# chathurawidanage/harp

Measured on AMD Instinct MI355X. Metric: sec/iteration K-means (N=1e8, d=100, K=1e4), lower is better.
Workload: dtype bf16; 1 GPU; model=kmeans-allreduce, N=100000000, d=100, K=10000, global_batch=100000000, parallelism=dp1

## Files before the change

csrc/kmeans_resolve.hip:

```cpp
#include "common.h"

namespace {

constexpr int KR_RUN = 2048;

template <int KS>
__global__ __launch_bounds__(64) __attribute__((amdgpu_waves_per_eu(3))) void kmeans_resolve_rowsum_kernel(
    const __bf16* __restrict__ X, long ldx, const __bf16* __restrict__ Cm2, const int* __restrict__ perm,
    const int* __restrict__ start, int NG, long n, int* __restrict__ labels, float* __restrict__ sums, int ld) {
  constexpr int DP = KS * 16;
  constexpr int NCB = (DP + 31) / 32;
  constexpr int STRE = NCB * 32 + 8;
  __shared__ __attribute__((aligned(16))) __bf16 tile[32 * STRE];
  __shared__ bf16x8 atile[KS * 64];
  const int lane = threadIdx.x;
  const int c = lane & 31, h = lane >> 5;
  const long j0 = (long)blockIdx.x * KR_RUN;
  if (j0 >= n) return;
  const long j1 = j0 + KR_RUN < n ? j0 + KR_RUN : n;

  for (int i = lane; i < 32 * STRE; i += 64) tile[i] = (__bf16)0.f;
  int lo = 0, hi = NG;
  while (hi - lo > 1) {
    const int mid = (lo + hi) >> 1;
    if (start[mid] <= j0) lo = mid; else hi = mid;
  }
  int k = lo;
  long kend = start[k + 1];
  int kloaded = -1;
  bool dirty = false;
  floatx16 S[NCB];
#pragma unroll
  for (int b = 0; b < NCB; ++b)
#pragma unroll
    for (int q = 0; q < 16; ++q) S[b][q] = 0.f;

  auto pos = [&](long jb) {
    const long j = jb + c;
    return j < j1 ? j : j1 - 1;
  };
  auto load_rows = [&](bf16x8 (&xf)[KS], int p) {
    const bf16x8* row = (const bf16x8*)(X + (long)p * ldx);
#pragma unroll
    for (int s = 0; s < KS; ++s) xf[s] = row[2 * s + h];
  };
  auto flush = [&](int kk) {
    float* o = sums + ((long)kk * 32 + 4 * h) * ld + c;
#pragma unroll
    for (int b = 0; b < NCB; ++b) {
#pragma unroll
      for (int q = 0; q < 16; ++q) {
        const int rq = (q & 3) + 8 * (q >> 2);
// ... 55 lines not shown
      int row = (mq & 3) + 8 * (mq >> 2) + 4 * h;
      const float om = __shfl_xor(m, 32, 64);
      const int orow = __shfl_xor(row, 32, 64);
      if (om < m || (om == m && orow < row)) row = orow;
      if (mine && h == 0) labels[pc] = k * 32 + row;
      const int code = mine ? row : -1;
#pragma unroll
      for (int t = 0; t < 2; ++t) {
        bf16x8 oh;
#pragma unroll
        for (int j = 0; j < 8; ++j) {
          const int r0 = __builtin_amdgcn_readlane(code, 16 * t + j), r1 = __builtin_amdgcn_readlane(code, 16 * t + 8 + j);
          oh[j] = (__bf16)((h ? r1 : r0) == c ? 1.f : 0.f);
        }
        const __bf16* tp = tile + (16 * t + 8 * h) * STRE + c;
#pragma unroll
        for (int b = 0; b < NCB; ++b) {
          bf16x8 xt;
#pragma unroll
          for (int j = 0; j < 8; ++j) xt[j] = tp[j * STRE + 32 * b];
          S[b] = __builtin_amdgcn_mfma_f32_32x32x16_bf16(oh, xt, S[b], 0, 0, 0);
          __builtin_amdgcn_sched_barrier(0);
        }
      }
      dirty = true;
      cur = sub_end;
    }
  }
  if (dirty) flush(k);
}

template <int KS>
int launch_resolve(const void* X, long ldx, const void* Cm2, const int* perm, const int* start, int NG, long n,
                   int* labels, float* sums, int ld, hipStream_t s) {
  const long nblk = (n + KR_RUN - 1) / KR_RUN;
  kmeans_resolve_rowsum_kernel<KS><<<dim3((unsigned)nblk), dim3(64), 0, s>>>(
      (const __bf16*)X, ldx, (const __bf16*)Cm2, perm, start, NG, n, labels, sums, ld);
  return harp_launch_status();
}

}

HARP_EXPORT int harp_kmeans_resolve_rowsum(const void* X, long ldx, const void* Cm2, int dp, const int* perm,
                                           const int* start, int NG, long n, int* labels, float* sums, int ld,
                                           hipStream_t s) {
  if (n <= 0) return n == 0 ? HARP_OK : HARP_EBADARG;
  if (dp <= 0 || dp % 16 || dp > 128 || ldx < dp || ldx % 8 || ld < dp || NG <= 0 || !labels || !sums)
    return HARP_EBADARG;
  switch (dp / 16) {
    case 1: return launch_resolve<1>(X, ldx, Cm2, perm, start, NG, n, labels, sums, ld, s);
    case 2: return launch_resolve<2>(X, ldx, Cm2, perm, start, NG, n, labels, sums, ld, s);
    case 3: return launch_resolve<3>(X, ldx, Cm2, perm, start, NG, n, labels, sums, ld, s);
    case 4: return launch_resolve<4>(X, ldx, Cm2, perm, start, NG, n, labels, sums, ld, s);
    case 5: return launch_resolve<5>(X, ldx, Cm2, perm, start, NG, n, labels, sums, ld, s);
    case 6: return launch_resolve<6>(X, ldx, Cm2, perm, start, NG, n, labels, sums, ld, s);
    case 7: return launch_resolve<7>(X, ldx, Cm2, perm, start, NG, n, labels, sums, ld, s);
    case 8: return launch_resolve<8>(X, ldx, Cm2, perm, start, NG, n, labels, sums, ld, s);
    default: return HARP_EUNSUPPORTED;
  }
}
```

csrc/segsum.hip:

```cpp
#include "common.h"

namespace {

constexpr int SEG = 64;

__global__ __launch_bounds__(256) void label_hist_kernel(const int* __restrict__ lab, long n, int K, long chunk,
                                                         int* __restrict__ H) {
  extern __shared__ __attribute__((aligned(16))) int hist[];
  for (int k = threadIdx.x; k < K; k += blockDim.x) hist[k] = 0;
  __syncthreads();
  const long a = (long)blockIdx.x * chunk;
  long b = a + chunk;
  if (b > n) b = n;
  for (long i = a + threadIdx.x; i < b; i += blockDim.x) atomicAdd(&hist[lab[i]], 1);
  __syncthreads();
  int* row = H + (long)blockIdx.x * K;
  for (int k = threadIdx.x; k < K; k += blockDim.x) row[k] = hist[k];
}

__global__ void colscan1_kernel(int* __restrict__ H, int nchunks, int K, int* __restrict__ T) {
  const int k = blockIdx.x * blockDim.x + threadIdx.x;
  const int s = blockIdx.y;
  if (k >= K) return;
  const int c0 = s * SEG;
  int c1 = c0 + SEG;
  if (c1 > nchunks) c1 = nchunks;
  int run = 0;
  for (int c = c0; c < c1; ++c) {
    const int v = H[(long)c * K + k];
    H[(long)c * K + k] = run;
    run += v;
  }
  T[(long)s * K + k] = run;
}

__global__ void colscan2_kernel(int* __restrict__ T, int nseg, int K, int* __restrict__ counts) {
  const int k = blockIdx.x * blockDim.x + threadIdx.x;
  if (k >= K) return;
  int run = 0;
  for (int s = 0; s < nseg; ++s) {
    const int v = T[(long)s * K + k];
    T[(long)s * K + k] = run;
    run += v;
  }
  counts[k] = run;
}

__global__ __launch_bounds__(1024) void segscan_kernel(const int* __restrict__ counts, int K, int* __restrict__ start) {
  __shared__ int part[1024];
  const int per = (K + 1023) / 1024;
  const int a = threadIdx.x * per;
  int s = 0;
  for (int j = 0; j < per; ++j)
    if (a + j < K) s += counts[a + j];
  part[threadIdx.x] = s;
  __syncthreads();
  for (int off = 1; off < 1024; off <<= 1) {
    const int v = threadIdx.x >= off ? part[threadIdx.x - off] : 0;
    __syncthreads();
    part[threadIdx.x] += v;
    __syncthreads();
  }
  int run = threadIdx.x ? part[threadIdx.x - 1] : 0;
  for (int j = 0; j < per; ++j)
    if (a + j < K) {
      start[a + j] = run;
      run += counts[a + j];
    }
  if (threadIdx.x == 1023) start[K] = part[1023];
}

__device__ __forceinline__ int xcd_contiguous(unsigned b, unsigned nb) {
  const unsigned q = nb / 8, r = nb % 8, x = b % 8;
  return (int)((x < r ? x * (q + 1) : r * (q + 1) + (x - r) * q) + b / 8);
}

__global__ __launch_bounds__(256) void bucket_kernel(const int* __restrict__ lab, long n, int K, long chunk,
                                                     const int* __restrict__ H, const int* __restrict__ T,
                                                     const int* __restrict__ start, int* __restrict__ perm) {
  extern __shared__ __attribute__((aligned(16))) int cur[];
  const int c = xcd_contiguous(blockIdx.x, gridDim.x), s = c / SEG;
  for (int k = threadIdx.x; k < K; k += blockDim.x)
    cur[k] = start[k] + T[(long)s * K + k] + H[(long)c * K + k];
  __syncthreads();
  const long a = (long)c * chunk;
  long b = a + chunk;
  if (b > n) b = n;
  constexpr int U = 8;
  for (long i0 = a + threadIdx.x; i0 < b; i0 += (long)U * blockDim.x) {
    int l[U];
#pragma unroll
    for (int u = 0; u < U; ++u) {
      const long i = i0 + (long)u * blockDim.x;
      l[u] = i < b ? lab[i] : -1;
    }
#pragma unroll
    for (int u = 0; u < U; ++u)
      if (l[u] >= 0) perm[atomicAdd(&cur[l[u]], 1)] = (int)(i0 + (long)u * blockDim.x);
  }
}

template <int LPR, int RUN, int ROWS = 4>
__global__ __launch_bounds__(256) void rowsum_bf16_kernel(const __bf16* __restrict__ X, int dp, long ldx,
                                                          const int* __restrict__ perm,
                                                          const int* __restrict__ start, int K, long n,
                                                          float* __restrict__ sums, int ld) {
  constexpr int SPW = 64 / LPR;
  const int lane = threadIdx.x & 63;
  const int sl = lane % LPR;
  const long slot = ((long)blockIdx.x * blockDim.x + threadIdx.x) / LPR;
  const long j0 = slot * RUN;
  if (j0 >= n) return;
  long j1 = j0 + RUN;
  if (j1 > n) j1 = n;
  const bool active = sl * 8 < dp;
  int lo = 0, hi = K;
  while (hi - lo > 1) {
    const int mid = (lo + hi) >> 1;
    if (start[mid] <= j0) lo = mid; else hi = mid;
// ... 102 lines not shown
        for (int c = 0; c < VEC; ++c)
          v[q][c] = active[c] ? *(const bf16x8*)(X + (long)pj[q] * ldx + (64 * c + lane) * 8) : bf16x8{};
#pragma unroll
      for (int c = 0; c < VEC; ++c)
#pragma unroll
        for (int q = 0; q < ROWS; q += 4)
#pragma unroll
          for (int e = 0; e < 8; ++e)
            acc[c][e] += ((float)v[q][c][e] + (float)v[q + 1][c][e]) + ((float)v[q + 2][c][e] + (float)v[q + 3][c][e]);
    }
    for (; j < stop; ++j) {
      const long r = perm[j];
#pragma unroll
      for (int c = 0; c < VEC; ++c) {
        if (active[c]) {
          const bf16x8 v = *(const bf16x8*)(X + r * ldx + (64 * c + lane) * 8);
#pragma unroll
          for (int e = 0; e < 8; ++e) acc[c][e] += (float)v[e];
        }
      }
    }
  }
  flush(k);
}

}

HARP_EXPORT long harp_bucket_chunk(long n) {
  long c = 65536;
  while (c > 4096 && (n + c - 1) / c < 1536) c >>= 1;
  return c;
}

HARP_EXPORT long harp_bucket_workspace_ints(long n, int K) {
  const long chunk = harp_bucket_chunk(n);
  const long nch = (n + chunk - 1) / chunk;
  const long nseg = (nch + SEG - 1) / SEG;
  return nch * K + nseg * K + K + (K + 1) + n;
}

HARP_EXPORT int harp_bucket_labels(const int* lab, long n, int K, int* ws, long* start_off, long* perm_off,
                                   hipStream_t s) {
  if (n <= 0 || K <= 0 || K > 16384) return HARP_EBADARG;
  const long chunk = harp_bucket_chunk(n);
  const int nch = (int)((n + chunk - 1) / chunk);
  const int nseg = (nch + SEG - 1) / SEG;
  int* H = ws;
  int* T = H + (long)nch * K;
  int* counts = T + (long)nseg * K;
  int* start = counts + K;
  int* perm = start + K + 1;
  *start_off = start - ws;
  *perm_off = perm - ws;
  const size_t lds = (size_t)K * sizeof(int);
  label_hist_kernel<<<dim3(nch), dim3(256), lds, s>>>(lab, n, K, chunk, H);
  colscan1_kernel<<<dim3((K + 255) / 256, nseg), dim3(256), 0, s>>>(H, nch, K, T);
  colscan2_kernel<<<dim3((K + 255) / 256), dim3(256), 0, s>>>(T, nseg, K, counts);
  segscan_kernel<<<dim3(1), dim3(1024), 0, s>>>(counts, K, start);
  bucket_kernel<<<dim3(nch), dim3(256), lds, s>>>(lab, n, K, chunk, H, T, start, perm);
  return harp_launch_status();
}

HARP_EXPORT int harp_bucket_rowsum_bf16(const void* X, int dp, long ldx, const int* perm, const int* start, int K,
                                        long n, float* sums, int ld, hipStream_t s) {
  if (dp % 8 || dp > 1024 || ld < dp || ldx < dp || ldx % 8 || n <= 0) return n == 0 ? HARP_OK : HARP_EBADARG;
  const int lpr_min = dp / 8;
  const __bf16* Xb = (const __bf16*)X;
  constexpr int RUN = 256;
  auto grid = [&](int lpr) { return dim3((unsigned)(((n + RUN - 1) / RUN * lpr + 255) / 256)); };
  if (lpr_min <= 8) rowsum_bf16_kernel<8, RUN><<<grid(8), dim3(256), 0, s>>>(Xb, dp, ldx, perm, start, K, n, sums, ld);
  else if (lpr_min <= 16) rowsum_bf16_kernel<16, RUN, 8><<<grid(16), dim3(256), 0, s>>>(Xb, dp, ldx, perm, start, K, n, sums, ld);
  else if (lpr_min <= 32) rowsum_bf16_kernel<32, RUN><<<grid(32), dim3(256), 0, s>>>(Xb, dp, ldx, perm, start, K, n, sums, ld);
  else if (dp <= 512) rowsum_wide_bf16_kernel<1, RUN><<<grid(64), dim3(256), 0, s>>>(Xb, dp, ldx, perm, start, K, n, sums, ld);
  else rowsum_wide_bf16_kernel<2, RUN><<<grid(64), dim3(256), 0, s>>>(Xb, dp, ldx, perm, start, K, n, sums, ld);
  return harp_launch_status();
}
```

harp_amd/ops/kmeans.py:

```python
from __future__ import annotations

import math
import os
from dataclasses import dataclass
from typing import Optional

import torch

from . import _lib, segment

KP_ALIGN = 128
ONES = 4
DEFAULT_VARIANT = 16
KEYLESS_VARIANT, KEYED_VARIANT = 16, 15
KEYLESS_MAX_DP = 128
RESOLVE_SPAN = 1 << 23


NARROW_MAX_DP = 256
WIDE_ALIGN = 64
WIDE_VARIANT = int(os.environ.get("HARP_KMEANS_WIDE_VARIANT", "0"))


def padded_dim(d: int) -> int:
    dp = (d + ONES + 15) // 16 * 16
    return dp if dp <= NARROW_MAX_DP else (d + ONES + WIDE_ALIGN - 1) // WIDE_ALIGN * WIDE_ALIGN


def padded_k(k: int) -> int:
    return (k + KP_ALIGN - 1) // KP_ALIGN * KP_ALIGN


def row_stride(dp: int) -> int:
    return (dp + 127) // 128 * 128


def pack_points(x: torch.Tensor, device: torch.device | str | None = None) -> torch.Tensor:
    device = torch.device(device) if device is not None else x.device
    n, d = x.shape
    dp = padded_dim(d)
    dt = torch.bfloat16 if device.type == "cuda" else torch.float32
    ld = row_stride(dp) if device.type == "cuda" else dp
    out = torch.zeros((n, ld), dtype=dt, device=device)
    out[:, :d] = x.to(device=device, dtype=dt)
    out[:, d:d + ONES] = 1.0
    return out[:, :dp]


def generate_points(n: int, d: int, lo: float = 0.0, hi: float = 1000.0, seed: int = 0,
# ... 90 lines not shown
    if want_objective and (obj_partial is None or obj_partial.numel() < nblk):
        obj_partial = torch.empty(nblk, dtype=torch.float32, device=dev)
    _lib.check(lib.harp_kmeans_wide_finish(keys.data_ptr(), n, labels.data_ptr(),
                                           obj_partial.data_ptr() if want_objective else None,
                                           min_dist.data_ptr() if min_dist is not None else None,
                                           _lib.stream_ptr(dev)), "kmeans_wide_finish")
    if sums is not None:
        _check_sums(sums, op, dev)
        perm, start = segment.bucket_labels(labels, op.Cm2.shape[0])
        segment.bucket_rowsum(X, perm, start, sums)
    obj = obj_partial[:nblk].double().sum() if want_objective else None
    return labels, obj


def assign(X: torch.Tensor, op: CentroidOperand, sums: Optional[torch.Tensor] = None,
           labels: Optional[torch.Tensor] = None, want_objective: bool = True, variant: int = DEFAULT_VARIANT,
           obj_partial: Optional[torch.Tensor] = None, accumulate: str = "bucket",
           min_dist: Optional[torch.Tensor] = None):
    n, dp = X.shape
    dev = X.device
    if labels is None:
        labels = torch.empty(n, dtype=torch.int32, device=dev)
    if _lib.use_native(X):
        lib = _lib.kernels()
        if dp > NARROW_MAX_DP:
            if accumulate == "atomic":
                raise ValueError("accumulate='atomic' is only fused into the narrow kernel (dp <= "
                                 f"{NARROW_MAX_DP}); the wide path (dp = {dp}) accumulates by bucket")
            return _assign_wide(X, op, sums, labels, want_objective, obj_partial, min_dist)
        keyless = (variant == KEYLESS_VARIANT and dp <= KEYLESS_MAX_DP and sums is not None
                   and accumulate == "bucket" and min_dist is None)
        if variant == KEYLESS_VARIANT and not keyless:
            variant = KEYED_VARIANT
        if dp > 128:
            variant = 4
        elif variant in (14, 15) and dp // 16 == 5:
            variant = 13
        ppb = lib.harp_kmeans_points_per_block(variant)
        if ppb <= 0:
            raise ValueError(f"unknown kmeans kernel variant {variant}")
        nblk = (n + ppb - 1) // ppb
        if want_objective and (obj_partial is None or obj_partial.numel() < nblk):
            obj_partial = torch.empty(nblk, dtype=torch.float32, device=dev)
        if sums is not None:
            _check_sums(sums, op, dev)
        _check_operands(X, op)
        fused = sums if accumulate == "atomic" else None
        bucket = sums is not None and fused is None
        chunks = pipeline_chunks(n, ppb) if bucket else 1
        per = max(1, (nblk + chunks - 1) // chunks) * ppb
        side = _side_stream(dev) if chunks > 1 else None
        main = torch.cuda.current_stream(dev)
        for r0 in range(0, n, per):
            r1 = min(n, r0 + per)
            b0 = r0 // ppb
            st = lib.harp_kmeans_assign(X[r0].data_ptr(), X.stride(0), op.Cm2.data_ptr(), r1 - r0, dp,
                                        swept_k(op), op.d,
                                        labels[r0].data_ptr(), _lib.ptr(fused),
                                        fused.stride(0) if fused is not None else 0,
                                        obj_partial[b0].data_ptr() if want_objective else None,
                                        min_dist[r0].data_ptr() if min_dist is not None else None, variant,
                                        _lib.stream_ptr(dev))
            _lib.check(st, "kmeans_assign")
            if not bucket:
                continue

            def bucket_sum(lab, Xc):
                if keyless:
                    for s0 in range(0, lab.numel(), RESOLVE_SPAN):
                        ls, Xs = lab[s0:s0 + RESOLVE_SPAN], Xc[s0:s0 + RESOLVE_SPAN]
                        perm, start = segment.bucket_labels(ls, swept_k(op) // 32)
                        segment.resolve_rowsum(Xs, op.Cm2, perm, start, ls, sums)
                else:
                    perm, start = segment.bucket_labels(lab, op.Cm2.shape[0])
                    segment.bucket_rowsum(Xc, perm, start, sums)

            if side is None:
                bucket_sum(labels, X)
                continue
            side.wait_stream(main)
            with torch.cuda.stream(side):
                bucket_sum(labels[r0:r1], X[r0:r1])
        if side is not None:
            main.wait_stream(side)
        obj = obj_partial[:nblk].double().sum() if want_objective else None
        return labels, obj
    Xf = X.float()
    d = op.d
    x = Xf[:, :d]
    C = -0.5 * op.Cm2[: op.K, :d].float()
    dist = op.cn[: op.K].unsqueeze(0) - 2.0 * (x @ C.t())
    lab = dist.argmin(1)
    labels.copy_(lab.to(labels.dtype))
    if min_dist is not None:
        min_dist.copy_((dist.gather(1, lab[:, None])[:, 0] + (x * x).sum(1)).to(min_dist.dtype))
    if sums is not None:
        sums[:, : d + 1].index_add_(0, lab, Xf[:, : d + 1])
    obj = None
    if want_objective:
        xs = (x.double() ** 2).sum(1)
        obj = (dist.gather(1, lab[:, None])[:, 0].double() + xs).clamp_min(0).sum()
    return labels, obj


def normalize(sums: torch.Tensor, c: torch.Tensor, d: int, counts: Optional[torch.Tensor] = None) -> torch.Tensor:
# ... 14 lines not shown
```

harp_amd/ops/segment.py:

```python
from __future__ import annotations

import ctypes
import os
from typing import Dict, Tuple

import torch

from . import _lib

_lib.register({
    "harp_bucket_chunk": [_lib.c_long],
    "harp_bucket_workspace_ints": [_lib.c_long, _lib.c_int],
    "harp_bucket_labels": [_lib.c_void_p, _lib.c_long, _lib.c_int, _lib.c_void_p, _lib.c_void_p, _lib.c_void_p,
                           _lib.c_void_p],
    "harp_bucket_rowsum_bf16": [_lib.c_void_p, _lib.c_int, _lib.c_long, _lib.c_void_p, _lib.c_void_p, _lib.c_int,
                                _lib.c_long, _lib.c_void_p, _lib.c_int, _lib.c_void_p],
    "harp_kmeans_resolve_rowsum": [_lib.c_void_p, _lib.c_long, _lib.c_void_p, _lib.c_int, _lib.c_void_p,
                                   _lib.c_void_p, _lib.c_int, _lib.c_long, _lib.c_void_p, _lib.c_void_p, _lib.c_int,
                                   _lib.c_void_p],
})
_WS: Dict[Tuple, torch.Tensor] = {}


def _lib_ret_long(fn):
    fn.restype = ctypes.c_long
    return fn


def bucket_labels(labels: torch.Tensor, K: int) -> Tuple[torch.Tensor, torch.Tensor]:
    n = labels.numel()
    if not _lib.use_native(labels):
        order = torch.argsort(labels.long(), stable=True)
        counts = torch.bincount(labels.long(), minlength=K)
        start = torch.zeros(K + 1, dtype=torch.int64)
        start[1:] = torch.cumsum(counts, 0)
        return order.to(torch.int32), start.to(torch.int32)
    lib = _lib.kernels()
    _lib_ret_long(lib.harp_bucket_workspace_ints)
    need = lib.harp_bucket_workspace_ints(n, K)
    stream = torch.cuda.current_stream(labels.device).cuda_stream
    key = (labels.device, n, K, stream)
    ws = _WS.get(key)
    if ws is None:
        ws = next((w for k, w in _WS.items() if k[0] == labels.device and k[3] == stream and w.numel() >= need),
                  None)
    if ws is None:
        for k in [k for k in _WS if k[3] == stream]:
            del _WS[k]
        ws = torch.empty(need, dtype=torch.int32, device=labels.device)
        _WS[key] = ws
    so, po = ctypes.c_long(0), ctypes.c_long(0)
    st = lib.harp_bucket_labels(labels.data_ptr(), n, K, ws.data_ptr(), ctypes.byref(so), ctypes.byref(po),
                                _lib.stream_ptr(labels.device))
    _lib.check(st, "bucket_labels")
    return ws[po.value:po.value + n], ws[so.value:so.value + K + 1]


SUM_SLICE = min(1024, max(8, int(os.environ.get("HARP_ROWSUM_SLICE", "1024")) // 8 * 8))


def bucket_rowsum(X: torch.Tensor, perm: torch.Tensor, start: torch.Tensor, out: torch.Tensor) -> torch.Tensor:
    K = start.numel() - 1
    if not _lib.use_native(X):
        idx = torch.repeat_interleave(torch.arange(K), (start[1:] - start[:-1]).long())
        out[:K, : X.shape[1]].index_add_(0, idx, X[perm.long()].float())
        return out
    assert X.dtype == torch.bfloat16 and X.stride(1) == 1 and out.dtype == torch.float32 and out.is_contiguous()
    for c0 in range(0, X.shape[1], SUM_SLICE):
        w = min(SUM_SLICE, X.shape[1] - c0)
        st = _lib.kernels().harp_bucket_rowsum_bf16(X[:, c0:].data_ptr(), w, X.stride(0), perm.data_ptr(),
                                                    start.data_ptr(), K, perm.numel(), out[:, c0:].data_ptr(),
                                                    out.stride(0), _lib.stream_ptr(X.device))
        _lib.check(st, "bucket_rowsum")
    return out


def resolve_rowsum(X: torch.Tensor, Cm2: torch.Tensor, perm: torch.Tensor, start: torch.Tensor,
                   labels: torch.Tensor, out: torch.Tensor) -> torch.Tensor:
    NG = start.numel() - 1
    dp = X.shape[1]
    assert X.dtype == torch.bfloat16 and X.stride(1) == 1 and out.dtype == torch.float32 and out.is_contiguous()
    assert Cm2.dtype == torch.bfloat16 and Cm2.is_contiguous() and Cm2.shape[1] == dp and Cm2.shape[0] >= 32 * NG
    assert out.shape[0] >= 32 * NG and labels.dtype == torch.int32 and labels.is_contiguous()
    assert labels.numel() == perm.numel() == X.shape[0]
    st = _lib.kernels().harp_kmeans_resolve_rowsum(X.data_ptr(), X.stride(0), Cm2.data_ptr(), dp, perm.data_ptr(),
                                                   start.data_ptr(), NG, perm.numel(), labels.data_ptr(),
                                                   out.data_ptr(), out.stride(0), _lib.stream_ptr(X.device))
    _lib.check(st, "kmeans_resolve_rowsum")
    return out
```

csrc/kmeans.hip:

```cpp
#include "common.h"

#include <atomic>
#include <type_traits>

namespace {

constexpr float KM_BIG = 1.0e38f;
constexpr int KM_ONES = 4;

__device__ __forceinline__ float keyed(float v, unsigned idx) {
  return __uint_as_float((__float_as_uint(v) & ~0xFu) | idx);
}

template <int KS, int G, int WAVES_, int RG>
struct KMCfg {
  static constexpr int DP = KS * 16;
  static constexpr int CPR = KS * 2;
  static constexpr int TILE = RG * 32;
  static constexpr int WAVES = WAVES_;
  static constexpr int THREADS = WAVES_ * 64;
  static constexpr int TILE_BYTES = TILE * DP * 2;
  static constexpr int DMA_INSTR = TILE * CPR / 64;
  static constexpr int PTS = WAVES_ * G * 32;
  static_assert((TILE * CPR) % 64 == 0, "tile must be whole 1-KiB DMA pieces");
// ... 10 lines not shown
      const int row = q / C::CPR;
      int c = q - row * C::CPR - ((row >> 3) & 1);
      if (c < 0) c += C::CPR;
      unsigned lo = (unsigned)(row * C::CPR + c) * 16u;
      asm("" : "+v"(lo));
      __builtin_amdgcn_global_load_lds((const void __attribute__((address_space(1)))*)(gsrc + (size_t)lo),
                                       (void __attribute__((address_space(3)))*)(lds + j * 1024), 16, 0, 0);
    }
  }
}

constexpr int km_ring_piece_at(int H, int i) {
  constexpr int at[2][4] = {{5, 7, 10, 13}, {6, 9, 11, 14}};
  for (int p = 0; p < 4; ++p)
    if (at[H][p] == i) return p;
  return -1;
}
constexpr int KM_RING_BARRIER_ITEM = 3;

template <int KS, int G, int WAVES, int RG, int PIPE, int PRIO = 0, int KEYLESS = 0, int RING = 0>
__global__ __launch_bounds__(WAVES * 64) void kmeans_assign_kernel(
    const __bf16* __restrict__ X, long ldx, const __bf16* __restrict__ Cm2, long N, int ntiles, int tail_rg,
    int dcount, int* __restrict__ labels, float* __restrict__ sums, int ld_sums, float* __restrict__ obj_partial,
    float* __restrict__ mind, long nblk, unsigned* __restrict__ next_block) {
  using C = KMCfg<KS, G, WAVES, RG>;
  constexpr int NSLOT = RING ? 3 : 2;
  static_assert(!RING || (KEYLESS && PIPE > 0 && G == 4 && RG == 4 && WAVES == 8 && KS <= 8),
                "the ring sweep is written for the keyless 4 x 4-item stage of 8 waves");
  __shared__ __attribute__((aligned(16))) char smem[NSLOT * C::TILE_BYTES + WAVES * 4 + 16];
  if constexpr (PRIO)
    if (__builtin_amdgcn_readfirstlane((int)threadIdx.x) >= WAVES * 32) __builtin_amdgcn_s_setprio(1);

  long b = blockIdx.x;
  while (b < nblk) {
    int tid = threadIdx.x;
    long nb = N;
    asm volatile("" : "+v"(tid), "+s"(nb));
    const int lane = tid & 63, wave = tid >> 6;
    const int r = lane & 31, h = lane >> 5;
    const int srot = (r >> 3) & 1;
    const int swave = __builtin_amdgcn_readfirstlane(wave);
    const long pbase = (b * WAVES + swave) * (G * 32);
    stage_dma<C>(Cm2, 0, smem, swave, lane);
    if constexpr (RING) stage_dma<C>(Cm2, ntiles > 1 ? 1 : 0, smem + C::TILE_BYTES, swave, lane);

    bf16x8 xf[G][KS];
#pragma unroll
    for (int g = 0; g < G; ++g) {
      long p = pbase + g * 32 + r;
      if (p > nb - 1) p = nb - 1;
      const bf16x8* row = (const bf16x8*)(X + p * ldx);
#pragma unroll
      for (int s = 0; s < KS; ++s) xf[g][s] = row[2 * s + h];
    }

    float best[G];
    int bestt[G];
#pragma unroll
    for (int g = 0; g < G; ++g) { best[g] = KM_BIG; bestt[g] = 0; }
    auto tile_argmin = [&](const floatx16& ac, int g, int tg) {
      if constexpr (KEYLESS) {
        float nb = best[g];
#pragma unroll
        for (int q = 0; q < 16; q += 2) nb = fminf(fminf(nb, ac[q]), ac[q + 1]);
        if (nb < best[g]) bestt[g] = tg;
        best[g] = nb;
      } else {
        float m = keyed(ac[0], 0u);
#pragma unroll
        for (int q = 1; q < 16; ++q) m = fminf(m, keyed(ac[q], (unsigned)q));
        if (m < best[g]) { best[g] = m; bestt[g] = tg; }
      }
    };

    int aoff[KS];
#pragma unroll
    for (int s = 0; s < KS; ++s) {
      int cp = 2 * s + h + srot;
      if (cp >= C::CPR) cp -= C::CPR;
      aoff[s] = (r * C::CPR + cp) * 16;
    }
    const int aoff0 = aoff[0], aoffL = aoff[KS - 1] - 32 * (KS - 1);
    auto a_frag = [&](const char* base, int s) {
      return *(const bf16x8*)(base + (s == KS - 1 ? aoffL : aoff0) + 32 * s);
    };

// ... 113 lines not shown
#pragma unroll
            for (int s = 0; s < KS; ++s) an = __builtin_amdgcn_mfma_f32_32x32x16_bf16(af[rg1 & 1][s], xf[g1][s], an, 0, 0, 0);
          }
          tile_argmin(acc[i & 1], g, t * RG + rg);
          if constexpr (PIPE == 2) {
#pragma unroll
            for (int s = 0; s < KS; ++s) {
              __builtin_amdgcn_sched_group_barrier(0x008, 1, 0);
              __builtin_amdgcn_sched_group_barrier(0x002, 4, 0);
            }
          }
        }
      } else
#pragma unroll
      for (int rg = 0; rg < RG; ++rg) {
        if (rg + 1 < RG) {
          const char* nb = buf + (rg + 1) * 32 * C::CPR * 16;
#pragma unroll
          for (int s = 0; s < KS; ++s) af[(rg + 1) & 1][s] = a_frag(nb, s);
        }
        const int tg = t * RG + rg;
#pragma unroll
        for (int g = 0; g < G; ++g) {
          floatx16 acc = {0.f, 0.f, 0.f, 0.f, 0.f, 0.f, 0.f, 0.f, 0.f, 0.f, 0.f, 0.f, 0.f, 0.f, 0.f, 0.f};
#pragma unroll
          for (int s = 0; s < KS; ++s)
            acc = __builtin_amdgcn_mfma_f32_32x32x16_bf16(af[rg & 1][s], xf[g][s], acc, 0, 0, 0);
          tile_argmin(acc, g, tg);
        }
      }
      asm volatile("s_waitcnt vmcnt(0)" ::: "memory");
      __syncthreads();
    }
    if (tail_rg) {
      const int t = ntiles - 1;
      const char* buf = smem + (t % NSLOT) * C::TILE_BYTES;
      for (int rg = 0; rg < tail_rg; ++rg) {
        const char* nb = buf + rg * 32 * C::CPR * 16;
        bf16x8 af[KS];
#pragma unroll
        for (int s = 0; s < KS; ++s) af[s] = a_frag(nb, s);
        const int tg = t * RG + rg;
#pragma unroll
        for (int g = 0; g < G; ++g) {
          floatx16 acc = {0.f, 0.f, 0.f, 0.f, 0.f, 0.f, 0.f, 0.f, 0.f, 0.f, 0.f, 0.f, 0.f, 0.f, 0.f, 0.f};
#pragma unroll
          for (int s = 0; s < KS; ++s) acc = __builtin_amdgcn_mfma_f32_32x32x16_bf16(af[s], xf[g][s], acc, 0, 0, 0);
          tile_argmin(acc, g, tg);
        }
      }
    }

    {
      int tid = threadIdx.x;
      asm volatile("" : "+v"(tid));
      const int lane = tid & 63, wave = tid >> 6, r = lane & 31, h = lane >> 5;
      unsigned* nextw = (unsigned*)(smem + NSLOT * C::TILE_BYTES + WAVES * 4);
      unsigned fetched = 0;
      if (tid == 0) fetched = gridDim.x + atomicAdd(next_block, 1u);
      auto lane_xor = [&](auto v, int o) {
        return __builtin_bit_cast(decltype(v), __builtin_amdgcn_ds_bpermute((lane ^ o) << 2, __builtin_bit_cast(int, v)));
      };
      int lab[G];
      float local_obj = 0.f;
#pragma unroll
      for (int g = 0; g < G; ++g) {
        float xs = 0.f;
#pragma unroll
        for (int s = 0; s < KS; ++s)
#pragma unroll
          for (int j = 0; j < 8; ++j) {
            const float v = (float)xf[g][s][j];
            xs = fmaf(v, v, xs);
          }
        xs += lane_xor(xs, 32);
        xs -= (float)KM_ONES;
        const float ob = lane_xor(best[g], 32);
        const int obt = lane_xor(bestt[g], 32);
        const bool take = KEYLESS ? (ob < best[g] || (ob == best[g] && obt < bestt[g]))
                                  : (h ? (ob <= best[g]) : (ob < best[g]));
        const float bv = take ? ob : best[g];
        const int bt = take ? obt : bestt[g];
        const int hw = take ? (1 - h) : h;
        const unsigned reg = __float_as_uint(bv) & 0xFu;
        const int idx = KEYLESS ? bt : bt * 32 + (int)(reg & 3u) + 8 * (int)(reg >> 2) + 4 * hw;
        lab[g] = idx;
        const long p = pbase + g * 32 + r;
        if (h == 0 && p < nb) {
          labels[p] = idx;
          const float bd = KEYLESS ? bv : __uint_as_float(__float_as_uint(bv) & ~0xFu);
          local_obj += fmaxf(bd + xs, 0.f);
          if (mind) mind[p] = bd + xs;
        }
      }
      if (obj_partial) {
        for (int o = 32; o > 0; o >>= 1) local_obj += lane_xor(local_obj, o);
        float* red = (float*)(smem + NSLOT * C::TILE_BYTES);
        if (lane == 0) red[wave] = local_obj;
        __syncthreads();
        if (tid == 0) {
          float acc = 0.f;
#pragma unroll
          for (int w = 0; w < WAVES; ++w) acc += red[w];
          obj_partial[b] = acc;
        }
      }

      if (!KEYLESS && sums) {
#pragma unroll
        for (int g = 0; g < G; ++g) {
          for (int i = 0; i < 32; ++i) {
            const long p = pbase + g * 32 + i;
            if (p >= nb) break;
            const int l = __shfl(lab[g], i, 64);
            const __bf16* xr = X + p * ldx;
            float* sr = sums + (long)l * ld_sums;
            for (int c = lane; c <= dcount; c += 64) atomicAdd(sr + c, (float)xr[c]);
          }
        }
      }
      if (tid == 0) *nextw = fetched;
      __syncthreads();
      b = (long)(unsigned)__builtin_amdgcn_readfirstlane((int)*nextw);
    }
  }
}

__global__ void kmeans_normalize_kernel(const float* __restrict__ sums, int ld, float* __restrict__ c,
                                        int Kr, int d, float* __restrict__ counts) {
  const int row = blockIdx.x * (blockDim.x >> 6) + (threadIdx.x >> 6);
  const int lane = threadIdx.x & 63;
  if (row >= Kr) return;
  const float cnt = sums[(long)row * ld + d];
  if (counts && lane == 0) counts[row] = cnt;
  if (cnt > 0.f) {
    const float inv = 1.0f / cnt;
    for (int j = lane; j < d; j += 64) c[(long)row * d + j] = sums[(long)row * ld + j] * inv;
  }
}

__global__ void kmeans_prepare_kernel(const float* __restrict__ c, int K, int d, int Kp, int dp,
                                      __bf16* __restrict__ Cm2, float* __restrict__ cn) {
  const int row = blockIdx.x * (blockDim.x >> 6) + (threadIdx.x >> 6);
  const int lane = threadIdx.x & 63;
  if (row >= Kp) return;
  float s = 0.f;
  for (int j = lane; j < d; j += 64) {
    float v = row < K ? c[(long)row * d + j] : 0.f;
    const float bf = (float)(__bf16)v;
    s = fmaf(bf, bf, s);
    Cm2[(long)row * dp + j] = (__bf16)(-2.0f * bf);
  }
  s = wave_sum(s);
  if (row >= K) s = KM_BIG;
  const __bf16 hi = (__bf16)s;
  const float r1 = s - (float)hi;
// ... 559 lines not shown
```

Before: 0.1336 s/iter.

## Bucket and resolve all label spans in single batched kernel launches

Replaces the Python loop over RESOLVE_SPAN chunks, which launched the five bucketing kernels plus one resolve kernel per span, with span-aware kernels that process every span in one launch. Each resolve block indexes its span's start offsets, and the scan kernels get a per-span grid dimension. The span also shrinks from 2^23 to 2^20 so buckets stay local to smaller windows. This cuts launch and host overhead and may improve locality of gathered rows. In exchange it adds more per-span start tables, more partial bucket flushes and atomics at span boundaries, and extra workspace.

```diff
diff --git a/csrc/kmeans_resolve.hip b/csrc/kmeans_resolve.hip
--- a/csrc/kmeans_resolve.hip
+++ b/csrc/kmeans_resolve.hip
@@ -7,7 +7,8 @@
 template <int KS>
 __global__ __launch_bounds__(64) __attribute__((amdgpu_waves_per_eu(3))) void kmeans_resolve_rowsum_kernel(
     const __bf16* __restrict__ X, long ldx, const __bf16* __restrict__ Cm2, const int* __restrict__ perm,
-    const int* __restrict__ start, int NG, long n, int* __restrict__ labels, float* __restrict__ sums, int ld) {
+    const int* __restrict__ start, int NG, long n, int span_shift, int* __restrict__ labels,
+    float* __restrict__ sums, int ld) {
   constexpr int DP = KS * 16;
   constexpr int NCB = (DP + 31) / 32;
   constexpr int STRE = NCB * 32 + 8;
@@ -18,6 +19,7 @@
   const long j0 = (long)blockIdx.x * KR_RUN;
   if (j0 >= n) return;
   const long j1 = j0 + KR_RUN < n ? j0 + KR_RUN : n;
+  start += (j0 >> span_shift) * (NG + 1);
 
   for (int i = lane; i < 32 * STRE; i += 64) tile[i] = (__bf16)0.f;
   int lo = 0, hi = NG;
@@ -139,30 +141,40 @@
 
 template <int KS>
 int launch_resolve(const void* X, long ldx, const void* Cm2, const int* perm, const int* start, int NG, long n,
-                   int* labels, float* sums, int ld, hipStream_t s) {
+                   int span_shift, int* labels, float* sums, int ld, hipStream_t s) {
   const long nblk = (n + KR_RUN - 1) / KR_RUN;
   kmeans_resolve_rowsum_kernel<KS><<<dim3((unsigned)nblk), dim3(64), 0, s>>>(
-      (const __bf16*)X, ldx, (const __bf16*)Cm2, perm, start, NG, n, labels, sums, ld);
+      (const __bf16*)X, ldx, (const __bf16*)Cm2, perm, start, NG, n, span_shift, labels, sums, ld);
   return harp_launch_status();
 }
 
 }
 
+HARP_EXPORT int harp_kmeans_resolve_run() { return KR_RUN; }
+
+HARP_EXPORT int harp_kmeans_resolve_rowsum_spans(const void* X, long ldx, const void* Cm2, int dp, const int* perm,
+                                                 const int* start, int NG, long n, long span, int* labels,
+                                                 float* sums, int ld, hipStream_t s) {
+  if (n <= 0) return n == 0 ? HARP_OK : HARP_EBADARG;
+  if (dp <= 0 || dp % 16 || dp > 128 || ldx < dp || ldx % 8 || ld < dp || NG <= 0 || !labels || !sums)
+    return HARP_EBADARG;
+  if (span < KR_RUN || (span & (span - 1))) return HARP_EBADARG;
+  const int sh = __builtin_ctzl((unsigned long)span);
+  switch (dp / 16) {
+    case 1: return launch_resolve<1>(X, ldx, Cm2, perm, start, NG, n, sh, labels, sums, ld, s);
+    case 2: return launch_resolve<2>(X, ldx, Cm2, perm, start, NG, n, sh, labels, sums, ld, s);
+    case 3: return launch_resolve<3>(X, ldx, Cm2, perm, start, NG, n, sh, labels, sums, ld, s);
+    case 4: return launch_resolve<4>(X, ldx, Cm2, perm, start, NG, n, sh, labels, sums, ld, s);
+    case 5: return launch_resolve<5>(X, ldx, Cm2, perm, start, NG, n, sh, labels, sums, ld, s);
+    case 6: return launch_resolve<6>(X, ldx, Cm2, perm, start, NG, n, sh, labels, sums, ld, s);
+    case 7: return launch_resolve<7>(X, ldx, Cm2, perm, start, NG, n, sh, labels, sums, ld, s);
+    case 8: return launch_resolve<8>(X, ldx, Cm2, perm, start, NG, n, sh, labels, sums, ld, s);
+    default: return HARP_EUNSUPPORTED;
+  }
+}
+
 HARP_EXPORT int harp_kmeans_resolve_rowsum(const void* X, long ldx, const void* Cm2, int dp, const int* perm,
                                            const int* start, int NG, long n, int* labels, float* sums, int ld,
                                            hipStream_t s) {
-  if (n <= 0) return n == 0 ? HARP_OK : HARP_EBADARG;
-  if (dp <= 0 || dp % 16 || dp > 128 || ldx < dp || ldx % 8 || ld < dp || NG <= 0 || !labels || !sums)
-    return HARP_EBADARG;
-  switch (dp / 16) {
-    case 1: return launch_resolve<1>(X, ldx, Cm2, perm, start, NG, n, labels, sums, ld, s);
-    case 2: return launch_resolve<2>(X, ldx, Cm2, perm, start, NG, n, labels, sums, ld, s);
-    case 3: return launch_resolve<3>(X, ldx, Cm2, perm, start, NG, n, labels, sums, ld, s);
-    case 4: return launch_resolve<4>(X, ldx, Cm2, perm, start, NG, n, labels, sums, ld, s);
-    case 5: return launch_resolve<5>(X, ldx, Cm2, perm, start, NG, n, labels, sums, ld, s);
-    case 6: return launch_resolve<6>(X, ldx, Cm2, perm, start, NG, n, labels, sums, ld, s);
-    case 7: return launch_resolve<7>(X, ldx, Cm2, perm, start, NG, n, labels, sums, ld, s);
-    case 8: return launch_resolve<8>(X, ldx, Cm2, perm, start, NG, n, labels, sums, ld, s);
-    default: return HARP_EUNSUPPORTED;
-  }
+  return harp_kmeans_resolve_rowsum_spans(X, ldx, Cm2, dp, perm, start, NG, n, 1L << 62, labels, sums, ld, s);
 }
diff --git a/csrc/segsum.hip b/csrc/segsum.hip
--- a/csrc/segsum.hip
+++ b/csrc/segsum.hip
@@ -3,6 +3,20 @@
 namespace {
 
 constexpr int SEG = 64;
+
+struct SpanGeom {
+  long chunk;
+  int nch;
+  int cps;
+  int sps;
+  int spans;
+};
+
+__host__ __device__ inline long ceil_pow2(long v) {
+  long p = 1;
+  while (p < v) p <<= 1;
+  return p;
+}
 
 __global__ __launch_bounds__(256) void label_hist_kernel(const int* __restrict__ lab, long n, int K, long chunk,
                                                          int* __restrict__ H) {
@@ -18,13 +32,15 @@
   for (int k = threadIdx.x; k < K; k += blockDim.x) row[k] = hist[k];
 }
 
-__global__ void colscan1_kernel(int* __restrict__ H, int nchunks, int K, int* __restrict__ T) {
+__global__ void colscan1_kernel(int* __restrict__ H, SpanGeom g, int K, int* __restrict__ T) {
   const int k = blockIdx.x * blockDim.x + threadIdx.x;
   const int s = blockIdx.y;
   if (k >= K) return;
-  const int c0 = s * SEG;
+  const int j = s / g.sps;
+  const int c0 = j * g.cps + (s % g.sps) * SEG;
   int c1 = c0 + SEG;
-  if (c1 > nchunks) c1 = nchunks;
+  if (c1 > (j + 1) * g.cps) c1 = (j + 1) * g.cps;
+  if (c1 > g.nch) c1 = g.nch;
   int run = 0;
   for (int c = c0; c < c1; ++c) {
     const int v = H[(long)c * K + k];
@@ -37,6 +53,8 @@
 __global__ void colscan2_kernel(int* __restrict__ T, int nseg, int K, int* __restrict__ counts) {
   const int k = blockIdx.x * blockDim.x + threadIdx.x;
   if (k >= K) return;
+  T += (long)blockIdx.y * nseg * K;
+  counts += (long)blockIdx.y * K;
   int run = 0;
   for (int s = 0; s < nseg; ++s) {
     const int v = T[(long)s * K + k];
@@ -46,8 +64,12 @@
   counts[k] = run;
 }
 
-__global__ __launch_bounds__(1024) void segscan_kernel(const int* __restrict__ counts, int K, int* __restrict__ start) {
+__global__ __launch_bounds__(1024) void segscan_kernel(const int* __restrict__ counts, int K, long span,
+                                                       int* __restrict__ start) {
   __shared__ int part[1024];
+  counts += (long)blockIdx.x * K;
+  start += (long)blockIdx.x * (K + 1);
+  const int base = (int)(blockIdx.x * span);
   const int per = (K + 1023) / 1024;
   const int a = threadIdx.x * per;
   int s = 0;
@@ -61,13 +83,13 @@
     part[threadIdx.x] += v;
     __syncthreads();
   }
-  int run = threadIdx.x ? part[threadIdx.x - 1] : 0;
+  int run = base + (threadIdx.x ? part[threadIdx.x - 1] : 0);
   for (int j = 0; j < per; ++j)
     if (a + j < K) {
       start[a + j] = run;
       run += counts[a + j];
     }
-  if (threadIdx.x == 1023) start[K] = part[1023];
+  if (threadIdx.x == 1023) start[K] = base + part[1023];
 }
 
 __device__ __forceinline__ int xcd_contiguous(unsigned b, unsigned nb) {
@@ -75,16 +97,17 @@
   return (int)((x < r ? x * (q + 1) : r * (q + 1) + (x - r) * q) + b / 8);
 }
 
-__global__ __launch_bounds__(256) void bucket_kernel(const int* __restrict__ lab, long n, int K, long chunk,
+__global__ __launch_bounds__(256) void bucket_kernel(const int* __restrict__ lab, long n, int K, SpanGeom g,
                                                      const int* __restrict__ H, const int* __restrict__ T,
                                                      const int* __restrict__ start, int* __restrict__ perm) {
   extern __shared__ __attribute__((aligned(16))) int cur[];
-  const int c = xcd_contiguous(blockIdx.x, gridDim.x), s = c / SEG;
+  const int c = xcd_contiguous(blockIdx.x, gridDim.x);
+  const int j = c / g.cps, s = j * g.sps + (c % g.cps) / SEG;
   for (int k = threadIdx.x; k < K; k += blockDim.x)
-    cur[k] = start[k] + T[(long)s * K + k] + H[(long)c * K + k];
+    cur[k] = start[(long)j * (K + 1) + k] + T[(long)s * K + k] + H[(long)c * K + k];
   __syncthreads();
-  const long a = (long)c * chunk;
-  long b = a + chunk;
+  const long a = (long)c * g.chunk;
+  long b = a + g.chunk;
   if (b > n) b = n;
   constexpr int U = 8;
   for (long i0 = a + threadIdx.x; i0 < b; i0 += (long)U * blockDim.x) {
@@ -253,33 +276,62 @@
   return c;
 }
 
+namespace {
+
+SpanGeom span_geom(long n, long span) {
+  SpanGeom g;
+  g.chunk = harp_bucket_chunk(n < span ? n : span);
+  if (g.chunk > span) g.chunk = span;
+  g.nch = (int)((n + g.chunk - 1) / g.chunk);
+  const long cps = span / g.chunk;
+  g.cps = (int)(cps < g.nch ? cps : g.nch);
+  g.sps = (g.cps + SEG - 1) / SEG;
+  g.spans = (int)((n + span - 1) / span);
+  return g;
+}
+
+long workspace_ints(const SpanGeom& g, long n, int K) {
+  return (long)g.nch * K + (long)g.spans * g.sps * K + (long)g.spans * K + (long)g.spans * (K + 1) + n;
+}
+
+bool span_ok(long span) { return span > 0 && (span & (span - 1)) == 0; }
+
+}
+
 HARP_EXPORT long harp_bucket_workspace_ints(long n, int K) {
-  const long chunk = harp_bucket_chunk(n);
-  const long nch = (n + chunk - 1) / chunk;
-  const long nseg = (nch + SEG - 1) / SEG;
-  return nch * K + nseg * K + K + (K + 1) + n;
-}
-
-HARP_EXPORT int harp_bucket_labels(const int* lab, long n, int K, int* ws, long* start_off, long* perm_off,
-                                   hipStream_t s) {
-  if (n <= 0 || K <= 0 || K > 16384) return HARP_EBADARG;
-  const long chunk = harp_bucket_chunk(n);
-  const int nch = (int)((n + chunk - 1) / chunk);
-  const int nseg = (nch + SEG - 1) / SEG;
+  return n > 0 ? workspace_ints(span_geom(n, ceil_pow2(n)), n, K) : 0;
+}
+
+HARP_EXPORT long harp_bucket_spans_workspace_ints(long n, int K, long span) {
+  if (!span_ok(span)) return -1;
+  return n > 0 ? workspace_ints(span_geom(n, span), n, K) : 0;
+}
+
+HARP_EXPORT int harp_bucket_labels_spans(const int* lab, long n, int K, long span, int* ws, long* start_off,
+                                         long* perm_off, hipStream_t s) {
+  if (n <= 0 || n > 0x7fffffffL || K <= 0 || K > 16384 || !span_ok(span)) return HARP_EBADARG;
+  const SpanGeom g = span_geom(n, span);
+  if ((long)g.spans * g.sps > 65535) return HARP_EUNSUPPORTED;
   int* H = ws;
-  int* T = H + (long)nch * K;
-  int* counts = T + (long)nseg * K;
-  int* start = counts + K;
-  int* perm = start + K + 1;
+  int* T = H + (long)g.nch * K;
+  int* counts = T + (long)g.spans * g.sps * K;
+  int* start = counts + (long)g.spans * K;
+  int* perm = start + (long)g.spans * (K + 1);
   *start_off = start - ws;
   *perm_off = perm - ws;
   const size_t lds = (size_t)K * sizeof(int);
-  label_hist_kernel<<<dim3(nch), dim3(256), lds, s>>>(lab, n, K, chunk, H);
-  colscan1_kernel<<<dim3((K + 255) / 256, nseg), dim3(256), 0, s>>>(H, nch, K, T);
-  colscan2_kernel<<<dim3((K + 255) / 256), dim3(256), 0, s>>>(T, nseg, K, counts);
-  segscan_kernel<<<dim3(1), dim3(1024), 0, s>>>(counts, K, start);
-  bucket_kernel<<<dim3(nch), dim3(256), lds, s>>>(lab, n, K, chunk, H, T, start, perm);
+  const unsigned kb = (K + 255) / 256;
+  label_hist_kernel<<<dim3(g.nch), dim3(256), lds, s>>>(lab, n, K, g.chunk, H);
+  colscan1_kernel<<<dim3(kb, g.spans * g.sps), dim3(256), 0, s>>>(H, g, K, T);
+  colscan2_kernel<<<dim3(kb, g.spans), dim3(256), 0, s>>>(T, g.sps, K, counts);
+  segscan_kernel<<<dim3(g.spans), dim3(1024), 0, s>>>(counts, K, span, start);
+  bucket_kernel<<<dim3(g.nch), dim3(256), lds, s>>>(lab, n, K, g, H, T, start, perm);
   return harp_launch_status();
+}
+
+HARP_EXPORT int harp_bucket_labels(const int* lab, long n, int K, int* ws, long* start_off, long* perm_off,
+                                   hipStream_t s) {
+  return harp_bucket_labels_spans(lab, n, K, ceil_pow2(n > 0 ? n : 1), ws, start_off, perm_off, s);
 }
 
 HARP_EXPORT int harp_bucket_rowsum_bf16(const void* X, int dp, long ldx, const int* perm, const int* start, int K,
diff --git a/harp_amd/ops/kmeans.py b/harp_amd/ops/kmeans.py
--- a/harp_amd/ops/kmeans.py
+++ b/harp_amd/ops/kmeans.py
@@ -14,7 +14,7 @@
 DEFAULT_VARIANT = 16
 KEYLESS_VARIANT, KEYED_VARIANT = 16, 15
 KEYLESS_MAX_DP = 128
-RESOLVE_SPAN = 1 << 23
+RESOLVE_SPAN = 1 << 20
 
 
 NARROW_MAX_DP = 256
@@ -171,6 +171,9 @@
                    and accumulate == "bucket" and min_dist is None)
         if variant == KEYLESS_VARIANT and not keyless:
             variant = KEYED_VARIANT
+        span = RESOLVE_SPAN
+        if keyless and (span < segment.resolve_run() or span & (span - 1)):
+            raise ValueError(f"RESOLVE_SPAN must be a power of two of at least {segment.resolve_run()}, got {span}")
         if dp > 128:
             variant = 4
         elif variant in (14, 15) and dp // 16 == 5:
@@ -206,10 +209,8 @@
 
             def bucket_sum(lab, Xc):
                 if keyless:
-                    for s0 in range(0, lab.numel(), RESOLVE_SPAN):
-                        ls, Xs = lab[s0:s0 + RESOLVE_SPAN], Xc[s0:s0 + RESOLVE_SPAN]
-                        perm, start = segment.bucket_labels(ls, swept_k(op) // 32)
-                        segment.resolve_rowsum(Xs, op.Cm2, perm, start, ls, sums)
+                    perm, start = segment.bucket_labels(lab, swept_k(op) // 32, span=span)
+                    segment.resolve_rowsum(Xc, op.Cm2, perm, start, lab, sums, span=span)
                 else:
                     perm, start = segment.bucket_labels(lab, op.Cm2.shape[0])
                     segment.bucket_rowsum(Xc, perm, start, sums)
diff --git a/harp_amd/ops/segment.py b/harp_amd/ops/segment.py
--- a/harp_amd/ops/segment.py
+++ b/harp_amd/ops/segment.py
@@ -2,7 +2,7 @@
 
 import ctypes
 import os
-from typing import Dict, Tuple
+from typing import Dict, Optional, Tuple
 
 import torch
 
@@ -13,11 +13,18 @@
     "harp_bucket_workspace_ints": [_lib.c_long, _lib.c_int],
     "harp_bucket_labels": [_lib.c_void_p, _lib.c_long, _lib.c_int, _lib.c_void_p, _lib.c_void_p, _lib.c_void_p,
                            _lib.c_void_p],
+    "harp_bucket_spans_workspace_ints": [_lib.c_long, _lib.c_int, _lib.c_long],
+    "harp_bucket_labels_spans": [_lib.c_void_p, _lib.c_long, _lib.c_int, _lib.c_long, _lib.c_void_p, _lib.c_void_p,
+                                 _lib.c_void_p, _lib.c_void_p],
     "harp_bucket_rowsum_bf16": [_lib.c_void_p, _lib.c_int, _lib.c_long, _lib.c_void_p, _lib.c_void_p, _lib.c_int,
                                 _lib.c_long, _lib.c_void_p, _lib.c_int, _lib.c_void_p],
     "harp_kmeans_resolve_rowsum": [_lib.c_void_p, _lib.c_long, _lib.c_void_p, _lib.c_int, _lib.c_void_p,
                                    _lib.c_void_p, _lib.c_int, _lib.c_long, _lib.c_void_p, _lib.c_void_p, _lib.c_int,
                                    _lib.c_void_p],
+    "harp_kmeans_resolve_run": [],
+    "harp_kmeans_resolve_rowsum_spans": [_lib.c_void_p, _lib.c_long, _lib.c_void_p, _lib.c_int, _lib.c_void_p,
+                                         _lib.c_void_p, _lib.c_int, _lib.c_long, _lib.c_long, _lib.c_void_p,
+                                         _lib.c_void_p, _lib.c_int, _lib.c_void_p],
 })
 _WS: Dict[Tuple, torch.Tensor] = {}
 
@@ -27,33 +34,45 @@
     return fn
 
 
-def bucket_labels(labels: torch.Tensor, K: int) -> Tuple[torch.Tensor, torch.Tensor]:
+def _one_span(n: int) -> int:
+    return 1 << max(0, n - 1).bit_length()
+
+
+def bucket_labels(labels: torch.Tensor, K: int, span: Optional[int] = None) -> Tuple[torch.Tensor, torch.Tensor]:
     n = labels.numel()
+    if span is not None and (span <= 0 or span & (span - 1)):
+        raise ValueError(f"span must be a power of two, got {span}")
     if not _lib.use_native(labels):
-        order = torch.argsort(labels.long(), stable=True)
-        counts = torch.bincount(labels.long(), minlength=K)
-        start = torch.zeros(K + 1, dtype=torch.int64)
-        start[1:] = torch.cumsum(counts, 0)
-        return order.to(torch.int32), start.to(torch.int32)
+        w = n if span is None else span
+        lab = labels.long()
+        order = torch.cat([s0 + torch.argsort(lab[s0:s0 + w], stable=True) for s0 in range(0, n, w)])
+        counts = torch.stack([torch.bincount(lab[s0:s0 + w], minlength=K) for s0 in range(0, n, w)])
+        start = torch.zeros((counts.shape[0], K + 1), dtype=torch.int64)
+        start[:, 1:] = torch.cumsum(counts, 1)
+        start += torch.arange(0, n, w)[:, None]
+        return order.to(torch.int32), (start[0] if span is None else start).to(torch.int32)
     lib = _lib.kernels()
-    _lib_ret_long(lib.harp_bucket_workspace_ints)
-    need = lib.harp_bucket_workspace_ints(n, K)
+    _lib_ret_long(lib.harp_bucket_spans_workspace_ints)
+    cspan = _one_span(n) if span is None else span
+    spans = (n + cspan - 1) // cspan
+    need = lib.harp_bucket_spans_workspace_ints(n, K, cspan)
     stream = torch.cuda.current_stream(labels.device).cuda_stream
-    key = (labels.device, n, K, stream)
+    key = (labels.device, n, K, cspan, stream)
     ws = _WS.get(key)
     if ws is None:
-        ws = next((w for k, w in _WS.items() if k[0] == labels.device and k[3] == stream and w.numel() >= need),
+        ws = next((w for k, w in _WS.items() if k[0] == labels.device and k[-1] == stream and w.numel() >= need),
                   None)
     if ws is None:
-        for k in [k for k in _WS if k[3] == stream]:
+        for k in [k for k in _WS if k[-1] == stream]:
             del _WS[k]
         ws = torch.empty(need, dtype=torch.int32, device=labels.device)
         _WS[key] = ws
     so, po = ctypes.c_long(0), ctypes.c_long(0)
-    st = lib.harp_bucket_labels(labels.data_ptr(), n, K, ws.data_ptr(), ctypes.byref(so), ctypes.byref(po),
-                                _lib.stream_ptr(labels.device))
+    st = lib.harp_bucket_labels_spans(labels.data_ptr(), n, K, cspan, ws.data_ptr(), ctypes.byref(so),
+                                      ctypes.byref(po), _lib.stream_ptr(labels.device))
     _lib.check(st, "bucket_labels")
-    return ws[po.value:po.value + n], ws[so.value:so.value + K + 1]
+    start = ws[so.value:so.value + spans * (K + 1)]
+    return ws[po.value:po.value + n], (start if span is None else start.view(spans, K + 1))
 
 
 SUM_SLICE = min(1024, max(8, int(os.environ.get("HARP_ROWSUM_SLICE", "1024")) // 8 * 8))
@@ -75,16 +94,23 @@
     return out
 
 
+def resolve_run() -> int:
+    return _lib.kernels().harp_kmeans_resolve_run()
+
+
 def resolve_rowsum(X: torch.Tensor, Cm2: torch.Tensor, perm: torch.Tensor, start: torch.Tensor,
-                   labels: torch.Tensor, out: torch.Tensor) -> torch.Tensor:
-    NG = start.numel() - 1
-    dp = X.shape[1]
+                   labels: torch.Tensor, out: torch.Tensor, span: Optional[int] = None) -> torch.Tensor:
+    n, dp = X.shape
+    NG = start.shape[-1] - 1
+    cspan = _one_span(max(n, resolve_run())) if span is None else span
     assert X.dtype == torch.bfloat16 and X.stride(1) == 1 and out.dtype == torch.float32 and out.is_contiguous()
     assert Cm2.dtype == torch.bfloat16 and Cm2.is_contiguous() and Cm2.shape[1] == dp and Cm2.shape[0] >= 32 * NG
     assert out.shape[0] >= 32 * NG and labels.dtype == torch.int32 and labels.is_contiguous()
-    assert labels.numel() == perm.numel() == X.shape[0]
-    st = _lib.kernels().harp_kmeans_resolve_rowsum(X.data_ptr(), X.stride(0), Cm2.data_ptr(), dp, perm.data_ptr(),
-                                                   start.data_ptr(), NG, perm.numel(), labels.data_ptr(),
-                                                   out.data_ptr(), out.stride(0), _lib.stream_ptr(X.device))
+    assert labels.numel() == perm.numel() == n
+    assert start.is_contiguous() and start.numel() == (n + cspan - 1) // cspan * (NG + 1)
+    st = _lib.kernels().harp_kmeans_resolve_rowsum_spans(X.data_ptr(), X.stride(0), Cm2.data_ptr(), dp,
+                                                         perm.data_ptr(), start.data_ptr(), NG, n, cspan,
+                                                         labels.data_ptr(), out.data_ptr(), out.stride(0),
+                                                         _lib.stream_ptr(X.device))
     _lib.check(st, "kmeans_resolve_rowsum")
     return out
```

New measurement: 0.1327 s/iter (median of 6 runs). Within noise of the previous version (-0.7%).

## Prefetch next block's points and first centroid tiles during epilogue

Applied to the files above, without the earlier changes.

In the persistent assign kernel, the next block index is now fetched with a relaxed atomic before the tail tiles are processed. The epilogue then starts the DMA of the first centroid tiles and the loads of the next block's X rows while the current block's labels and objective are still being written. This hides the per-block startup latency of the X loads and tile staging. It also skips the squared-norm computation when neither objective nor min-distance output is requested. The cost is higher register pressure from the live xf array across iterations and an extra barrier placed earlier in the epilogue.

```diff
diff --git a/csrc/kmeans.hip b/csrc/kmeans.hip
--- a/csrc/kmeans.hip
+++ b/csrc/kmeans.hip
@@ -66,6 +66,28 @@
     if (__builtin_amdgcn_readfirstlane((int)threadIdx.x) >= WAVES * 32) __builtin_amdgcn_s_setprio(1);
 
   long b = blockIdx.x;
+  bf16x8 xf[G][KS];
+  constexpr bool EARLY = KS <= 8;
+  auto load_x = [&](int g, long blk, int sw, int r, int h, long nb) {
+    long p = (blk * WAVES + sw) * (G * 32) + g * 32 + r;
+    if (p > nb - 1) p = nb - 1;
+    const bf16x8* row = (const bf16x8*)(X + p * ldx);
+#pragma unroll
+    for (int s = 0; s < KS; ++s) xf[g][s] = row[2 * s + h];
+  };
+  auto first_tiles = [&](int sw, int lane) {
+    stage_dma<C>(Cm2, 0, smem, sw, lane);
+    if constexpr (RING) stage_dma<C>(Cm2, ntiles > 1 ? 1 : 0, smem + C::TILE_BYTES, sw, lane);
+  };
+  if (EARLY && b < nblk) {
+    int tid = threadIdx.x;
+    long nb = N;
+    asm volatile("" : "+v"(tid), "+s"(nb));
+    const int lane = tid & 63, sw = __builtin_amdgcn_readfirstlane(tid >> 6);
+    first_tiles(sw, lane);
+#pragma unroll
+    for (int g = 0; g < G; ++g) load_x(g, b, sw, lane & 31, lane >> 5, nb);
+  }
   while (b < nblk) {
     int tid = threadIdx.x;
     long nb = N;
@@ -75,17 +97,10 @@
     const int srot = (r >> 3) & 1;
     const int swave = __builtin_amdgcn_readfirstlane(wave);
     const long pbase = (b * WAVES + swave) * (G * 32);
-    stage_dma<C>(Cm2, 0, smem, swave, lane);
-    if constexpr (RING) stage_dma<C>(Cm2, ntiles > 1 ? 1 : 0, smem + C::TILE_BYTES, swave, lane);
-
-    bf16x8 xf[G][KS];
-#pragma unroll
-    for (int g = 0; g < G; ++g) {
-      long p = pbase + g * 32 + r;
-      if (p > nb - 1) p = nb - 1;
-      const bf16x8* row = (const bf16x8*)(X + p * ldx);
-#pragma unroll
-      for (int s = 0; s < KS; ++s) xf[g][s] = row[2 * s + h];
+    if constexpr (!EARLY) {
+      first_tiles(swave, lane);
+#pragma unroll
+      for (int g = 0; g < G; ++g) load_x(g, b, swave, r, h, nb);
     }
 
     float best[G];
@@ -265,6 +280,13 @@
       asm volatile("s_waitcnt vmcnt(0)" ::: "memory");
       __syncthreads();
     }
+    unsigned fetched;
+    if (EARLY && threadIdx.x == 0) {
+      typedef __attribute__((address_space(1))) unsigned gunsigned;
+      gunsigned* word = (gunsigned*)next_block;
+      asm volatile("" : "+v"(word));
+      fetched = __hip_atomic_fetch_add(word, 1u, __ATOMIC_RELAXED, __HIP_MEMORY_SCOPE_AGENT);
+    }
     if (tail_rg) {
       const int t = ntiles - 1;
       const char* buf = smem + (t % NSLOT) * C::TILE_BYTES;
@@ -289,8 +311,19 @@
       asm volatile("" : "+v"(tid));
       const int lane = tid & 63, wave = tid >> 6, r = lane & 31, h = lane >> 5;
       unsigned* nextw = (unsigned*)(smem + NSLOT * C::TILE_BYTES + WAVES * 4);
-      unsigned fetched = 0;
-      if (tid == 0) fetched = gridDim.x + atomicAdd(next_block, 1u);
+      long bnext = 0;
+      bool more = false;
+      const int sw = __builtin_amdgcn_readfirstlane(wave);
+      if constexpr (EARLY) {
+        if (tid == 0) *nextw = gridDim.x + fetched;
+        __syncthreads();
+        bnext = (long)(unsigned)__builtin_amdgcn_readfirstlane((int)*nextw);
+        more = bnext < nblk;
+        if (more) first_tiles(sw, lane);
+      } else if (tid == 0) {
+        fetched = atomicAdd(next_block, 1u);
+      }
+      const bool want_dist = obj_partial || mind;
       auto lane_xor = [&](auto v, int o) {
         return __builtin_bit_cast(decltype(v), __builtin_amdgcn_ds_bpermute((lane ^ o) << 2, __builtin_bit_cast(int, v)));
       };
@@ -299,15 +332,18 @@
 #pragma unroll
       for (int g = 0; g < G; ++g) {
         float xs = 0.f;
-#pragma unroll
-        for (int s = 0; s < KS; ++s)
-#pragma unroll
-          for (int j = 0; j < 8; ++j) {
-            const float v = (float)xf[g][s][j];
-            xs = fmaf(v, v, xs);
-          }
-        xs += lane_xor(xs, 32);
-        xs -= (float)KM_ONES;
+        if (want_dist) {
+#pragma unroll
+          for (int s = 0; s < KS; ++s)
+#pragma unroll
+            for (int j = 0; j < 8; ++j) {
+              const float v = (float)xf[g][s][j];
+              xs = fmaf(v, v, xs);
+            }
+          xs += lane_xor(xs, 32);
+          xs -= (float)KM_ONES;
+        }
+        if (EARLY && more) load_x(g, bnext, sw, r, h, nb);
         const float ob = lane_xor(best[g], 32);
         const int obt = lane_xor(bestt[g], 32);
         const bool take = KEYLESS ? (ob < best[g] || (ob == best[g] && obt < bestt[g]))
@@ -352,9 +388,12 @@
           }
         }
       }
-      if (tid == 0) *nextw = fetched;
-      __syncthreads();
-      b = (long)(unsigned)__builtin_amdgcn_readfirstlane((int)*nextw);
+      if constexpr (!EARLY) {
+        if (tid == 0) *nextw = gridDim.x + fetched;
+        __syncthreads();
+        bnext = (long)(unsigned)__builtin_amdgcn_readfirstlane((int)*nextw);
+      }
+      b = bnext;
     }
   }
 }
```

Result: no change. 0.1328 s/iter before, 0.1320 s/iter after, median of 6 (-0.6%).
